# Siyou-Li/u2Tokenizer

Hardware: AMD Instinct MI355X
Metric: CT volumes/sec (256^3 fp16) through u2Tokenizer fwd (higher is better)
Workload: dtype bf16; 1 GPU; BASELINE configs[2]: u2Qwen3-8B-shaped path, 256^3 volume = 8x(32,256,256) fp16, ViT-B 3D x12, SPP, 4-layer rma+diffts+dmtp tokenizer (8 heads, top_k 1024, scales {1,2,4}, 256 queries), text 1024, prompt 1024; hidden_size=4096, batch_per_gpu=1, streams_per_gpu=2, parallelism=replicas x1, tta_side_stream=off in the multi-stream run, on in the one-stream run

## Files before the change

include/u2tok.h:

```cpp
#ifndef U2TOK_H_
#define U2TOK_H_

#include <stddef.h>
#include <stdint.h>

#ifdef __cplusplus
extern "C" {
#endif

#define U2TOK_OK 0
#define U2TOK_ERR_ARG (-1)
#define U2TOK_ERR_LAUNCH (-2)
#define U2TOK_ERR_WORKSPACE (-3)
#define U2TOK_ERR_DEVICE (-4)

typedef void* u2tok_stream_t;

int u2tok_version(void);
const char* u2tok_arch(void);
const char* u2tok_elem(void);
int u2tok_device_check(void);
typedef struct u2tok_ctx* u2tok_ctx_t;
int u2tok_ctx_create(u2tok_ctx_t* out);
int u2tok_ctx_destroy(u2tok_ctx_t ctx);
// ... 33 lines not shown
  int32_t layer_num;
} u2tok_spp_config;

typedef struct {
  int32_t B;
  int32_t T;
  int32_t N;
  int32_t E;
  int32_t Lt;
  int32_t num_heads;
  int32_t num_layers;
  int32_t top_k;
  int32_t num_query;
  int32_t use_multi_scale;
  int32_t attn_type;
  int32_t enable_diffts;
  int32_t enable_dmtp;
  int32_t max_seq_len;
  float diffts_tau;
  float ln_eps;
} u2tok_tokenizer_config;

#define U2TOK_TOK_NW(layers) (1 + 18 * (layers) + 4 + 33 * (layers) + 9)


size_t u2tok_vit_workspace_bytes(const u2tok_vit_config* cfg);
int u2tok_vit_forward(const u2tok_vit_config* cfg, const void* const* weights, const void* volume, void* out,
                      void* workspace, size_t workspace_bytes, u2tok_stream_t stream);

size_t u2tok_spp_workspace_bytes(const u2tok_spp_config* cfg);
int u2tok_spp_forward(const u2tok_spp_config* cfg, const void* const* weights, const void* x, void* out,
                      void* workspace, size_t workspace_bytes, u2tok_stream_t stream);

size_t u2tok_tokenizer_workspace_bytes(const u2tok_tokenizer_config* cfg);
int u2tok_tokenizer_forward(const u2tok_tokenizer_config* cfg, const void* const* weights, const void* v_token,
                            const void* t_token, void* out, int64_t* topk_idx_out, void* svr_out, void* workspace,
                            size_t workspace_bytes, u2tok_stream_t stream);

typedef struct {
  const void* const* svr_in;
  void* const* svr_out;
  const void* visual_in;
  void* visual_out;
  const void* const* tta_in;
  void* const* tta_out;
} u2tok_tokenizer_taps;
int u2tok_tokenizer_forward_taps(const u2tok_tokenizer_config* cfg, const void* const* weights, const void* v_token,
                                 const void* t_token, void* out, int64_t* topk_idx_out, const u2tok_tokenizer_taps* taps,
                                 void* workspace, size_t workspace_bytes, u2tok_stream_t stream);

int u2tok_embed_splice(const void* table, const int64_t* ids, const void* feats, void* out, int32_t B, int32_t S,
                       int32_t E, int32_t nfeat, int64_t vocab, u2tok_stream_t stream);

size_t u2tok_preprocess_workspace_bytes(int32_t D, int32_t H, int32_t W);
int u2tok_preprocess_volume(const float* vol, void* out, int32_t* info, int32_t D, int32_t H, int32_t W, int32_t target,
                            int32_t depth_pad, float lower_pct, float upper_pct, int32_t out_dtype, void* workspace,
                            size_t workspace_bytes, u2tok_stream_t stream);

typedef struct {
  int32_t rot90_k;
// ... 252 lines not shown
```

u2tokenizer_amd/_lib.py:

```python
from __future__ import annotations

import ctypes as C
import os
import subprocess
import threading
from pathlib import Path

_PKG = Path(__file__).resolve().parent
_LIB = _PKG / "lib" / "libu2tok_hip.so"
_LIBS = {"bf16": _LIB, "f16": _PKG / "lib" / "libu2tok_hip_f16.so"}
_lock = threading.Lock()
_handles = {}


class LibraryNotBuilt(RuntimeError):
    pass


def lib_path() -> Path:
    return _LIB


def build(verbose: bool = False) -> Path:
    cmd = ["make", "-C", str(_PKG / "csrc"), "-j", str(os.cpu_count() or 4)]
# ... 72 lines not shown
_vp, _i32, _i64, _f32, _sz = C.c_void_p, C.c_int32, C.c_int64, C.c_float, C.c_size_t

SIGNATURES = {
    "u2tok_version": (_i32, []),
    "u2tok_arch": (C.c_char_p, []),
    "u2tok_elem": (C.c_char_p, []),
    "u2tok_device_check": (_i32, []),
    "u2tok_ctx_create": (_i32, [C.POINTER(_vp)]),
    "u2tok_ctx_destroy": (_i32, [_vp]),
    "u2tok_ctx_set_current": (_i32, [_vp]),
    "u2tok_ctx_get_current": (_vp, []),
    "u2tok_set_option": (_i32, [C.c_char_p, _i32]),
    "u2tok_profile_collect": (_i32, [_vp, _vp, _vp, _i32]),
    "u2tok_profile_collect2": (_i32, [_vp, _vp, _vp, _vp, _i32]),
    "u2tok_set_gemm_scratch": (_i32, [_vp, _sz, _vp]),
    "u2tok_vit_workspace_bytes": (_sz, [C.POINTER(VitConfig)]),
    "u2tok_vit_forward": (_i32, [C.POINTER(VitConfig), C.POINTER(_vp), _vp, _vp, _vp, _sz, _vp]),
    "u2tok_spp_workspace_bytes": (_sz, [C.POINTER(SppConfig)]),
    "u2tok_spp_forward": (_i32, [C.POINTER(SppConfig), C.POINTER(_vp), _vp, _vp, _vp, _sz, _vp]),
    "u2tok_tokenizer_workspace_bytes": (_sz, [C.POINTER(TokConfig)]),
    "u2tok_tokenizer_forward": (_i32, [C.POINTER(TokConfig), C.POINTER(_vp), _vp, _vp, _vp, _vp, _vp, _vp, _sz, _vp]),
    "u2tok_tokenizer_forward_taps": (_i32, [C.POINTER(TokConfig), C.POINTER(_vp), _vp, _vp, _vp, _vp, C.POINTER(TokTaps),
                                            _vp, _sz, _vp]),
    "u2tok_tok_attention_workspace_bytes": (_sz, [_i32, _i32, _i32, _i32, _i32]),
    "u2tok_tok_attention": (_i32, [_vp, _vp, _vp, _vp, _i32, _i32, _i32, _i32, _i32, _i64, _i64, _i64, _i64, _i64, _i64, _i64,
                                   _i64, _f32, _vp, _i32, _i32, _vp, _sz, _vp]),
    "u2tok_preprocess_workspace_bytes": (_sz, [_i32, _i32, _i32]),
    "u2tok_preprocess_volume": (_i32, [_vp, _vp, _vp, _i32, _i32, _i32, _i32, _i32, _f32, _f32, _i32, _vp, _sz, _vp]),
    "u2tok_preprocess_volume_aug": (_i32, [_vp, _vp, _vp, _i32, _i32, _i32, _i32, _i32, _f32, _f32, _i32,
                                           C.POINTER(Augment), _vp, _sz, _vp]),
    "u2tok_embed_splice": (_i32, [_vp, _vp, _vp, _vp, _i32, _i32, _i32, _i32, _i64, _vp]),
    "u2tok_gemm_bf16": (_i32, [_vp, _vp, _vp, _vp, _vp, _i32, _i32, _i32, _i64, _i64, _i64, _i64, _i32, _i32,
                               _i64, _i64, _i64, _i64, _i64, _i64, _i64, _i64, _f32, _i32, _vp]),
    "u2tok_layernorm_bf16": (_i32, [_vp, _vp, _vp, _vp, _vp, _i32, _i32, _f32, _vp]),
    "u2tok_layernorm_rows": (_i32, [_vp, _vp, _vp, _vp, _vp, _i32, _i32, _i32, _i64, _i64, _i64, _i64, _i64, _i64, _f32, _vp]),
    "u2tok_softmax_rows": (_i32, [_vp, _vp, _i32, _i32, _i32, _i64, _i64, _f32, _vp, _i32, _i32, _vp]),
    "u2tok_transpose_bf16": (_i32, [_vp, _vp, _i32, _i32, _i32, _i64, _i64, _i64, _i64, _i32, _vp]),
    "u2tok_im2col_patches": (_i32, [_vp, _i32, _vp, _i32, _i32, _i32, _i32, _i32, _i32, _i32, _vp]),
    "u2tok_avgpool3d_tokens": (_i32, [_vp, _vp, _i32, _i32, _i32, _i32, _i32, _i32, _i32, _i32, _vp]),
    "u2tok_score_gemv": (_i32, [_vp, _vp, _vp, _vp, _i32, _i32, _vp]),
    "u2tok_topk_sorted": (_i32, [_vp, _vp, _i32, _i32, _i32, _vp]),
    "u2tok_gather_rows": (_i32, [_vp, _vp, _vp, _i32, _i32, _i32, _i32, _vp]),
    "u2tok_multiscale_pool": (_i32, [_vp, _vp, _i32, _i32, _i32, _vp, _vp, _vp, _vp]),
    "u2tok_temporal_attention": (_i32, [_vp, _vp, _vp, _vp, _i32, _i32, _i32, _i32, _i32, _i64, _i64, _f32, _vp,
                                        _i32, _vp]),
    "u2tok_flash_attention_d64": (_i32, [_vp, _vp, _vp, _vp, _i32, _i32, _i32, _i64, _i64, _i64, _i64, _i32, _f32,
# ... 131 lines not shown
```

u2tokenizer_amd/csrc/capi.hip:

```cpp
#include <math.h>
#include <string.h>
#include <new>
#include <vector>
#include "pipeline.h"

using namespace u2;

static_assert(U2TOK_OK == U2_OK && U2TOK_ERR_ARG == U2_ERR_ARG && U2TOK_ERR_LAUNCH == U2_ERR_LAUNCH &&
                  U2TOK_ERR_WORKSPACE == U2_ERR_WORKSPACE && U2TOK_ERR_DEVICE == U2_ERR_DEVICE,
              "public and internal status codes must agree");

#define BF(p) reinterpret_cast<const bf16_t*>(p)
#define BFW(p) reinterpret_cast<bf16_t*>(p)
#define ST(s) reinterpret_cast<hipStream_t>(s)

extern "C" {

int u2tok_version(void) { return 200;  }
const char* u2tok_arch(void) { return "gfx950"; }
const char* u2tok_elem(void) { return U2_ELEM_ASM; }

int u2tok_device_check(void) {
  int dev = 0;
  if (hipGetDevice(&dev) != hipSuccess) return U2_ERR_DEVICE;
// ... 14 lines not shown
  delete cx;
  return U2_OK;
}
int u2tok_ctx_set_current(u2tok_ctx_t c) {
  ctx_bind(reinterpret_cast<Context*>(c));
  return U2_OK;
}
u2tok_ctx_t u2tok_ctx_get_current(void) { return reinterpret_cast<u2tok_ctx_t>(ctx_bound()); }

int u2tok_set_option(const char* name, int value) {
  if (!name) return U2_ERR_ARG;
  Options& o = ctx().opt;
  struct Opt { const char* name; int Options::*field; int lo, hi; };
  static const Opt table[] = {
      {"gemm_splitk", &Options::gemm_splitk, -1, 16},   {"gemm_mubuf", &Options::gemm_mubuf, 0, 1}, {"ln_wide", &Options::ln_wide, 0, 1},   {"gemm_big", &Options::gemm_big, -1, 27},
      {"gemm_big_grid", &Options::gemm_big_grid, 1, 4096}, {"gemm_big_splitk", &Options::gemm_big_splitk, 0, 16},
      {"gemm_big_drain", &Options::gemm_big_drain, 0, 1}, {"gemm_skinny", &Options::gemm_skinny, 0, 2},
       {"kmajor_b", &Options::kmajor_b, 0, 1},            {"gemm_tail_fused", &Options::gemm_tail_fused, 0, 1},
      {"flash_mode", &Options::flash_mode, 0, 7},        {"flash_q_prescaled", &Options::flash_q_prescaled, 0, 1},
      {"vit_flash", &Options::vit_flash, 0, 1},         {"tta_overlap", &Options::tta_overlap, 0, 1},
      {"vit_vt_epilogue", &Options::vit_vt_epilogue, 0, 1},
      {"tok_flash", &Options::tok_flash, 0, 1},
      {"tok_wide", &Options::tok_wide, 0, 2},
  };
  if (!strcmp(name, "gemm_tile")) {
    if (value != 0 && value != 64 && value != 128) return U2_ERR_ARG;
    o.gemm_tile = value;
    return U2_OK;
  }
  if (!strcmp(name, "profile")) { prof_enable(value != 0); return U2_OK; }
  for (const Opt& t : table)
    if (!strcmp(name, t.name)) {
      if (value < t.lo || value > t.hi) return U2_ERR_ARG;
      if (t.field == &Options::gemm_big && value > 0 && !(value >= 20 && value <= 27 && value != 23 && value != 25)) return U2_ERR_ARG;
      if (t.field == &Options::flash_mode && value != 0 && value != 1 && value != 7) return U2_ERR_ARG;
      o.*(t.field) = value;
      return U2_OK;
    }
  return U2_ERR_ARG;
}

int u2tok_set_gemm_scratch(void* device_ptr, size_t bytes, void* stream) {
  ctx().set_scratch(reinterpret_cast<hipStream_t>(stream), device_ptr, device_ptr ? bytes : 0);
  return U2_OK;
}

// ... 31 lines not shown
}

size_t u2tok_tokenizer_workspace_bytes(const u2tok_tokenizer_config* cfg) {
  if (!cfg) return 0;
  size_t peak = 0;
  if (tokenizer_forward(*cfg, nullptr, nullptr, nullptr, nullptr, nullptr, nullptr, nullptr, nullptr, 0, true, &peak,
                        nullptr) != U2_OK)
    return 0;
  return peak + 256;
}
int u2tok_tokenizer_forward(const u2tok_tokenizer_config* cfg, const void* const* weights, const void* v_token,
                            const void* t_token, void* out, int64_t* topk_idx_out, void* svr_out, void* workspace,
                            size_t workspace_bytes, u2tok_stream_t stream) {
  if (!cfg || !workspace || ((uintptr_t)workspace & 255)) return U2_ERR_ARG;
  return tokenizer_forward(*cfg, weights, BF(v_token), BF(t_token), BFW(out), topk_idx_out, BFW(svr_out), nullptr, workspace,
                           workspace_bytes, false, nullptr, ST(stream));
}
int u2tok_tokenizer_forward_taps(const u2tok_tokenizer_config* cfg, const void* const* weights, const void* v_token,
                                 const void* t_token, void* out, int64_t* topk_idx_out, const u2tok_tokenizer_taps* taps,
                                 void* workspace, size_t workspace_bytes, u2tok_stream_t stream) {
  if (!cfg || !taps || !workspace || ((uintptr_t)workspace & 255)) return U2_ERR_ARG;
  return tokenizer_forward(*cfg, weights, BF(v_token), BF(t_token), BFW(out), topk_idx_out, nullptr, taps, workspace,
                           workspace_bytes, false, nullptr, ST(stream));
}

size_t u2tok_preprocess_workspace_bytes(int32_t D, int32_t H, int32_t W) { return preprocess_workspace_bytes(D, H, W); }
int u2tok_preprocess_volume(const float* vol, void* out, int32_t* info, int32_t D, int32_t H, int32_t W, int32_t target,
                            int32_t depth_pad, float lower_pct, float upper_pct, int32_t out_dtype, void* workspace,
                            size_t workspace_bytes, u2tok_stream_t stream) {
  return preprocess_volume(vol, out, info, D, H, W, target, depth_pad, lower_pct, upper_pct, out_dtype, nullptr, workspace,
                           workspace_bytes, ST(stream));
}
int u2tok_preprocess_volume_aug(const float* vol, void* out, int32_t* info, int32_t D, int32_t H, int32_t W, int32_t target,
                                int32_t depth_pad, float lower_pct, float upper_pct, int32_t out_dtype,
                                const u2tok_augment* aug, void* workspace, size_t workspace_bytes, u2tok_stream_t stream) {
  if (!aug) return U2_ERR_ARG;
  PreAugment a;
  a.rot_k = aug->rot90_k;
  for (int i = 0; i < 3; ++i) a.flip[i] = aug->flip[i];
  a.mul = 1.0f + aug->scale_factor;
  a.add = aug->shift_offset;
  return preprocess_volume(vol, out, info, D, H, W, target, depth_pad, lower_pct, upper_pct, out_dtype, &a, workspace,
                           workspace_bytes, ST(stream));
}

int u2tok_embed_splice(const void* table, const int64_t* ids, const void* feats, void* out, int32_t B, int32_t S,
// ... 493 lines not shown
```

u2tokenizer_amd/csrc/ctx.h:

```cpp
#pragma once
#include <mutex>
#include <vector>
#include "common.h"

namespace u2 {

struct Options {
  int ln_wide = 1;
  int gemm_tile = 0;
  int gemm_mubuf = 1;
  int gemm_splitk = 0;
  int gemm_big = 0;
  int gemm_big_grid = 256;
  int gemm_big_splitk = 0;
  int gemm_big_drain = 1;
  int gemm_skinny = 2;
  int gemm_tail_fused = 1;
  int kmajor_b = 1;
  int flash_mode = 0;
  int flash_q_prescaled = 0;
  int vit_flash = 1;
  int vit_vt_epilogue = 1;
  int tok_flash = 1;
  int tok_wide = 2;
  int tta_overlap = 1;
  int profile = 0;
};

struct SideStream {
  hipStream_t owner = nullptr;
  hipStream_t s = nullptr;
  hipEvent_t fork = nullptr;
  hipEvent_t done[16] = {};
};

struct Scratch {
  hipStream_t st;
  void* p;
  size_t bytes;
};

struct ProfRec {
  hipEvent_t a, b;
  int cat;
  double flops, bytes;
};

struct Context {
// ... 22 lines not shown
```

u2tokenizer_amd/csrc/pipeline.h:

```cpp
#pragma once
#include <algorithm>
#include "../../include/u2tok.h"
#include "kernels.h"

namespace u2 {

typedef u2tok_vit_config VitConfig;
typedef u2tok_spp_config SppConfig;
typedef u2tok_tokenizer_config TokConfig;
typedef u2tok_tokenizer_taps TokTaps;

inline int layernorm_dense(const bf16_t* x, const bf16_t* res, const bf16_t* w, const bf16_t* b, bf16_t* y, int rows, int C,
                           float eps, hipStream_t st) {
  return layernorm_bf16(x, res, w, b, y, 1, rows, C, 0, C, 0, C, 0, C, eps, st);
}

int vit_forward(const VitConfig& c, const void* const* W, const void* volume, bf16_t* out, void* ws, size_t ws_bytes,
                bool dry, size_t* peak, hipStream_t st);
int spp_forward(const SppConfig& c, const void* const* W, const bf16_t* x, bf16_t* out, void* ws, size_t ws_bytes,
                bool dry, size_t* peak, hipStream_t st);
int tokenizer_forward(const TokConfig& c, const void* const* W, const bf16_t* v_token, const bf16_t* t_token,
                      bf16_t* out, int64_t* topk_idx_out, bf16_t* svr_out, const TokTaps* taps, void* ws, size_t ws_bytes,
                      bool dry, size_t* peak, hipStream_t st);

}
```

u2tokenizer_amd/csrc/pipeline.hip:

```cpp
#include <vector>
#include "pipeline.h"

namespace u2 {

namespace {

struct Arena {
  char* base;
  size_t cap;
  size_t off = 0, peak = 0;
  bool dry;
  Arena(void* b, size_t c, bool d) : base((char*)b), cap(c), dry(d) {}
  template <typename T>
  T* get(size_t count) {
    const size_t a = (off + 255) & ~(size_t)255;
    off = a + count * sizeof(T);
    if (off > peak) peak = off;
    if (dry) return reinterpret_cast<T*>((uintptr_t)0x1000 + a);
    return (off <= cap) ? reinterpret_cast<T*>(base + a) : nullptr;
  }
  bool ok() const { return dry || peak <= cap; }
};

struct ScratchScope {
// ... 258 lines not shown
  Arena ar(ws, ws_bytes, dry);
  const Run r{ar, dry, st};
  bf16_t* pooled = ar.get<bf16_t>((size_t)rows * c.in_dim);
  bf16_t* ha = ar.get<bf16_t>((size_t)rows * c.out_dim);
  bf16_t* hb = ar.get<bf16_t>((size_t)rows * c.out_dim);
  U2_CHECK_WS(ar);
  U2_RUN(avgpool3d_tokens(x, pooled, c.nchunk, g1, g2, g3, w1, w2, w3, c.in_dim, st));
  const bf16_t* cur = pooled;
  int cur_dim = c.in_dim;
  for (int l = 0; l < c.layer_num; ++l) {
    const bool last = (l == c.layer_num - 1);
    bf16_t* dst = last ? out : ((l & 1) ? hb : ha);
    U2_TRY(linear(r, cur, {w[2 * l], w[2 * l + 1]}, dst, c.out_dim, rows, cur_dim, c.out_dim,
                  (!last && c.layer_type == 0) ? GEMM_GELU : 0));
    cur = dst;
    cur_dim = c.out_dim;
  }
  if (peak) *peak = ar.peak;
  return U2_OK;
}

namespace {
struct Att { Lin q, k, v, o; const bf16_t* rb; };
struct SvrLayer { Att spatial, temporal; };
struct TtaLayer { Att self, visual, text; Lin norm_self, norm_v, norm_t; };
struct TokWeights {
  const bf16_t* query;
  Lin score, gate;
  Att linagg;
  std::vector<SvrLayer> svr;
  std::vector<TtaLayer> tta;
};
TokWeights tok_weights(const TokConfig& c, Table t) {
  auto att = [&](int i, bool self) {
    return Att{{t[i], t[i + 1]}, {t[i + 2], t[i + 3]}, {t[i + 4], t[i + 5]}, {t[i + 6], t[i + 7]}, self && c.attn_type == 0 ? t[i + 8] : nullptr};
  };
  const int L = c.num_layers, i_sel = 1 + 18 * L, i_tta = i_sel + 4, i_lin = i_tta + 33 * L;
  TokWeights w{t[0], {t[i_sel], t[i_sel + 1]}, {nullptr, nullptr}, att(i_lin, false), {}, {}};
  if (c.enable_dmtp) w.gate = {t[i_sel + 2], t[i_sel + 3]};
  for (int l = 0, i = 1; l < L; ++l, i += 18) w.svr.push_back({att(i, true), att(i + 9, true)});
  for (int l = 0, i = i_tta; l < L; ++l, i += 33)
    w.tta.push_back({att(i, true), att(i + 9, false), att(i + 18, false), {t[i + 27], t[i + 28]}, {t[i + 29], t[i + 30]}, {t[i + 31], t[i + 32]}});
  return w;
}

int packed_proj(const Run& r, const bf16_t* x, std::initializer_list<Lin> p, bf16_t* out, int64_t rows, int E) {
  const Lin* l = p.begin(); const int n = (int)p.size();
  bool packed = l[0].w && l[0].b;
  for (int i = 1; i < n; ++i) packed = packed && l[i].w == l[i - 1].w + (size_t)E * E && l[i].b == l[i - 1].b + E;
  if (packed) return linear(r, x, l[0], out, n * E, rows, E, n * E);
  for (int i = 0; i < n; ++i) U2_TRY(linear(r, x, l[i], out + i * E, n * E, rows, E, E));
  return U2_OK;
}
int rope_qk(const Run& r, const Heads& hd, bf16_t* qkv, int64_t n_outer, int S, int n_inner) {
  const int E = hd.H * hd.d;
  U2_RUN(rope_apply(qkv, n_outer, S, n_inner, hd.H, hd.d, 3 * E, hd.max_len, 0, r.st));
  U2_RUN(rope_apply(qkv + E, n_outer, S, n_inner, hd.H, hd.d, 3 * E, hd.max_len, 0, r.st));
  return U2_OK;
}
template <typename P> inline P* slot(P* const* per_layer, int l) { return per_layer ? per_layer[l] : nullptr; }

struct Tok {
  const TokConfig& c; Run r; const TokWeights& w;
  TokTaps taps;
  const bf16_t* t_token;
  int B, T, N, E, L, Q, k;
  Heads hd;
  int64_t rows, qrows;
  bf16_t *xa, *xb, *qkv, *sctx;
  const bf16_t* V; int Lv;
  bf16_t *qa, *qb, *qc, *qproj, *qctx, *qo;
  SideStream* side; bool overlap;
  bf16_t *kv_inline, *kv_v[8], *kv_t[8], *k_lin;

  int temporal_across_batch() {
    const size_t mark = r.ar.off;
    bf16_t* g = r.ar.get<bf16_t>((size_t)rows * 3 * E);
    bf16_t* gc = r.ar.get<bf16_t>((size_t)rows * E);
    U2_CHECK_WS(r.ar);
    const size_t S2 = (size_t)B * N;
    for (int b = 0; b < B; ++b)
      U2_TRY(copy_runs(r, g + (size_t)b * N * 3 * E, S2 * 3 * E, qkv + (size_t)b * T * N * 3 * E, (size_t)N * 3 * E, (size_t)N * 3 * E, T));
    U2_TRY(self_attention(r, hd, g, gc, T, (int)S2, 3 * E, (int64_t)S2 * 3 * E, nullptr));
    for (int b = 0; b < B; ++b)
      U2_TRY(copy_runs(r, sctx + (size_t)b * T * N * E, (size_t)N * E, gc + (size_t)b * N * E, S2 * E, (size_t)N * E, T));
    r.ar.off = mark;
    return U2_OK;
  }

  int svr_layer(int l, const bf16_t*& x) {
    const SvrLayer& a = w.svr[l];
    if (const void* in = slot(taps.svr_in, l)) x = reinterpret_cast<const bf16_t*>(in);
    bf16_t* y = (x == xa) ? xb : xa;
    U2_TRY(packed_proj(r, x, {a.spatial.q, a.spatial.k, a.spatial.v}, qkv, rows, E));
    if (c.attn_type == 1) U2_TRY(rope_qk(r, hd, qkv, (int64_t)B * T, N, 1));
    if (c.attn_type == 2)
      U2_TRY(chunk_axis_attention(r, hd, qkv, sctx, 1, B * T, N, a.spatial.rb));
    else
      U2_TRY(self_attention(r, hd, qkv, sctx, B * T, N, 3 * E, (int64_t)N * 3 * E, a.spatial.rb));
    U2_TRY(linear(r, sctx, a.spatial.o, y, E, rows, E, E));
    bf16_t* y2 = (y == xa) ? xb : xa;
    U2_TRY(packed_proj(r, y, {a.temporal.q, a.temporal.k, a.temporal.v}, qkv, rows, E));
    if (c.attn_type == 1) U2_TRY(rope_qk(r, hd, qkv, B, T, N));
    if (c.attn_type == 2 && B == 1)
      U2_TRY(self_attention(r, hd, qkv, sctx, T, N, 3 * E, (int64_t)N * 3 * E, a.temporal.rb));
    else if (c.attn_type == 2)
      U2_TRY(temporal_across_batch());
    else
      U2_TRY(chunk_axis_attention(r, hd, qkv, sctx, B, T, N, a.temporal.rb));
    U2_TRY(linear(r, sctx, a.temporal.o, y2, E, rows, E, E));
    x = y2;
    return tap(r, slot(taps.svr_out, l), x, (size_t)rows * E);
  }

  int select_diffts(const bf16_t* x, bf16_t* sel) {
    const int TN = T * N;
    const size_t mark = r.ar.off;
    const int64_t ldS = round_up(TN, 8);
    float* scT = r.ar.get<float>((size_t)B * k * ldS);
    bf16_t* P = r.ar.get<bf16_t>((size_t)B * k * ldS);
    const bool x_in_place = opts().kmajor_b && !(TN & 7);
    bf16_t* Xt = x_in_place ? nullptr : r.ar.get<bf16_t>((size_t)B * E * ldS);
    U2_CHECK_WS(r.ar);
    {
      GemmDesc g;
      g.A = w.score.w; g.B = x; g.C = scT; g.bias = w.score.b;
      g.M = k; g.N = TN; g.K = E; g.lda = E; g.ldb = E; g.ldc = ldS;
      g.nz = B; g.sBb = (int64_t)TN * E; g.sCb = (int64_t)k * ldS;
      g.flags = GEMM_BIAS_M | GEMM_OUT_F32;
      U2_RUN(gemm_bf16(g, r.st));
    }
    U2_RUN(softmax_rows(scT, P, B, k, TN, ldS, ldS, (int64_t)k * ldS, (int64_t)k * ldS, 1.0f / c.diffts_tau, nullptr, 1, 0, r.st));
    {
      GemmDesc g;
// ... 105 lines not shown
  }

  int linear_aggregation(const bf16_t* qcur, bf16_t* out) {
    U2_TRY(linear(r, qcur, w.linagg.q, qproj, E, qrows, E, E));
    if (overlap)
      U2_RUN(hip_status(hipStreamWaitEvent(r.st, side->done[2 * L], 0)));
    else
      U2_TRY(linear(r, V, w.linagg.k, k_lin, E, (int64_t)B * Lv, E, E));
    return cross_attention(r, hd, qproj, k_lin, V, E, out, B, Q, Lv);
  }
};
}

int tokenizer_forward(const TokConfig& c, const void* const* W, const bf16_t* v_token, const bf16_t* t_token,
                      bf16_t* out, int64_t* topk_idx_out, bf16_t* svr_out, const TokTaps* taps, void* ws, size_t ws_bytes,
                      bool dry, size_t* peak, hipStream_t st) {
  if (c.B <= 0 || c.T <= 0 || c.N <= 0 || c.E <= 0 || c.Lt <= 0 || c.num_heads <= 0 || c.num_layers < 0) return U2_ERR_ARG;
  if (c.E % c.num_heads || (c.E / c.num_heads) % 8 || c.top_k <= 0 || c.num_query <= 0) return U2_ERR_ARG;
  if (c.attn_type < 0 || c.attn_type > 2) return U2_ERR_ARG;
  if (!dry && (!W || !v_token || !t_token || !out)) return U2_ERR_ARG;
  const int B = c.B, E = c.E, d = E / c.num_heads, L = c.num_layers, k = c.top_k;
  if (!c.enable_diffts && k > c.T * c.N) return U2_ERR_ARG;
  if (c.N > c.max_seq_len || c.T > c.max_seq_len || c.num_query > c.max_seq_len) return U2_ERR_ARG;
  const TokWeights w = tok_weights(c, Table{dry ? nullptr : W});

  Arena ar(ws, ws_bytes, dry);
  const size_t kSplitK = std::max<size_t>(24u << 20, (size_t)16 * B * c.num_query * 3 * E);
  char* skw = ar.get<char>(kSplitK);
  U2_CHECK_WS(ar);
  ScratchScope scratch_scope(ctx(), st, skw, kSplitK, !dry);
  Tok t{c, Run{ar, dry, st}, w, (taps && !dry) ? *taps : TokTaps{}, t_token, B, c.T, c.N, E, L, c.num_query, k,
        Heads{c.num_heads, d, 1.0f / sqrtf((float)d), c.max_seq_len}, (int64_t)B * c.T * c.N, (int64_t)B * c.num_query};
  const Run& r = t.r;
  t.xa = ar.get<bf16_t>((size_t)t.rows * E);
  t.xb = ar.get<bf16_t>((size_t)t.rows * E);
  t.qkv = ar.get<bf16_t>((size_t)t.rows * 3 * E);
  t.sctx = ar.get<bf16_t>((size_t)t.rows * E);
  U2_CHECK_WS(ar);

  const bf16_t* x = v_token;
  for (int l = 0; l < L; ++l) U2_TRY(t.svr_layer(l, x));
  U2_TRY(tap(r, svr_out, x, (size_t)t.rows * E));
  bf16_t* sel = ar.get<bf16_t>((size_t)B * k * E);
  U2_CHECK_WS(ar);
  U2_TRY(c.enable_diffts ? t.select_diffts(x, sel) : t.select_topk(x, sel, topk_idx_out));
  U2_TRY(t.multiscale_pooling(sel));
  U2_TRY(t.tta_prefetch());
  U2_RUN(fill_rows(w.query, t.qa, B, (int64_t)t.Q * E, (int64_t)t.Q * E, st));
  bf16_t* qcur = t.qa;
  for (int l = 0; l < L; ++l) U2_TRY(t.tta_layer(l, qcur));
  U2_TRY(t.linear_aggregation(qcur, out));
  if (peak) *peak = ar.peak;
  U2_CHECK_WS(ar);
  return U2_OK;
}

}
```

u2tokenizer_amd/tokenizer.py:

```python
from __future__ import annotations

import ctypes as C

import torch
import torch.nn as nn

from . import _lib, ops

_ATTN_TYPES = {"rma": 0, "rope": 1}


def _init_attn(m):
    for lin in (m.wq, m.wk, m.wv, m.dense):
        nn.init.xavier_uniform_(lin.weight)
        if lin.bias is not None:
            nn.init.zeros_(lin.bias)


class RelativeMultiheadAttention(nn.Module):

    def __init__(self, d_model, num_heads, max_seq_len=512):
        super().__init__()
        assert d_model % num_heads == 0
        self.num_heads, self.d_model, self.depth, self.max_seq_len = num_heads, d_model, d_model // num_heads, max_seq_len
# ... 138 lines not shown
def _pack_qkv_linear(m) -> None:
    ws, bs = [m.wq.weight, m.wk.weight, m.wv.weight], [m.wq.bias, m.wk.bias, m.wv.bias]
    E = ws[0].shape[0]
    step_w, step_b = ws[0].numel() * ws[0].element_size(), bs[0].numel() * bs[0].element_size()
    if all(w.is_contiguous() for w in ws) and all(ws[i + 1].data_ptr() == ws[i].data_ptr() + step_w for i in (0, 1)) \
            and all(bs[i + 1].data_ptr() == bs[i].data_ptr() + step_b for i in (0, 1)):
        return
    W = torch.cat([w.data for w in ws], 0).contiguous()
    Bv = torch.cat([b.data for b in bs], 0).contiguous()
    for i in range(3):
        ws[i].data = W[i * E:(i + 1) * E]
        bs[i].data = Bv[i * E:(i + 1) * E]


def _att_ptrs(m, value_side: bool = True):
    if not value_side:
        return [m.wq.weight, m.wq.bias, m.wk.weight, m.wk.bias, None, None, None, None, None]
    if isinstance(m, nn.MultiheadAttention):
        E = m.embed_dim
        W, b = m.in_proj_weight, m.in_proj_bias
        return [W[:E], b[:E], W[E:2 * E], b[E:2 * E], W[2 * E:], b[2 * E:], m.out_proj.weight, m.out_proj.bias, None]
    return [m.wq.weight, m.wq.bias, m.wk.weight, m.wk.bias, m.wv.weight, m.wv.bias, m.dense.weight, m.dense.bias,
            getattr(m, "relative_bias", None)]


def _unshare_packed(module, state_dict, prefix, local_metadata):
    for k, v in list(state_dict.items()):
        if k.startswith(prefix) and torch.is_tensor(v) and \
                v.untyped_storage().nbytes() != v.numel() * v.element_size():
            state_dict[k] = v.detach().clone() if not v.requires_grad else v.clone().detach()
    return state_dict


class u2Tokenizer(nn.Module):

    def __init__(self, embed_size, num_heads, num_layers, top_k, use_multi_scale, num_3d_query_token, hidden_size,
                 attn_type="rma", enable_diffts=False, enable_dmtp=False):
        super().__init__()
        if embed_size != hidden_size:
            raise ValueError("embed_size must equal hidden_size (builder.py:5,11 pass config.hidden_size for both)")
        self.svt_module = SpatioTemporalVisualTokenRefinerModel(
            embed_size=embed_size, num_heads=num_heads, num_layers=num_layers, top_k=top_k,
            use_multi_scale=use_multi_scale, attn_type=attn_type, enable_diffts=enable_diffts,
            enable_dmtp=enable_dmtp)
        self.tta_module = TextConditionTokenAggregatorModel(d_model=embed_size, num_layers=num_layers,
                                                            num_heads=num_heads, attn_type=attn_type)
        self.query_tokens = nn.Parameter(torch.zeros(1, num_3d_query_token, hidden_size))
        self.query_tokens.data.normal_(mean=0.0, std=0.02)
        self.embed_size, self.num_heads, self.num_layers, self.top_k = embed_size, num_heads, num_layers, top_k
        self.use_multi_scale, self.num_query, self.attn_type = bool(use_multi_scale), num_3d_query_token, attn_type
        self.enable_diffts, self.enable_dmtp = bool(enable_diffts), bool(enable_dmtp)
        self._ws = ops._Workspace()
        self._packed_key = None
        self._dead_offloaded = False
        self._register_state_dict_hook(_unshare_packed)
        self.last_topk_indices = None
        self.capture_svr_tokens = False
        self.last_svr_tokens = None

    def _weights(self):
        w = [self.query_tokens]
        for layer in self.svt_module.attention_network.layers:
            w += _att_ptrs(layer.spatial_attention) + _att_ptrs(layer.temporal_attention)
        sn = self.svt_module.token_selection.score_net
        w += [sn.weight, sn.bias]
        if self.enable_dmtp:
            w += [self.svt_module.dynamic_pool.gate_fc.weight, self.svt_module.dynamic_pool.gate_fc.bias]
        else:
            w += [None, None]
        for layer in self.tta_module.layers_vt:
            w += _att_ptrs(layer.self_attention) + _att_ptrs(layer.visual_cross_attention) \
                + _att_ptrs(layer.text_cross_attention)
            w += [layer.norm_self.weight, layer.norm_self.bias, layer.norm_cross_v.weight, layer.norm_cross_v.bias,
                  layer.norm_cross_t.weight, layer.norm_cross_t.bias]
        w += _att_ptrs(self.tta_module.layer_linagg.linear_aggregator, value_side=False)
        return w

    def pack_weights(self) -> None:
        key = (self.query_tokens.data_ptr(), self.query_tokens.dtype)
        if self._packed_key == key:
            return
        with torch.no_grad():
            for layer in self.svt_module.attention_network.layers:
                _pack_qkv(layer.spatial_attention)
                _pack_qkv(layer.temporal_attention)
            for layer in self.tta_module.layers_vt:
                for m in (layer.self_attention, layer.visual_cross_attention, layer.text_cross_attention):
                    _pack_qkv(m)
        if self.query_tokens.is_cuda:
            torch.cuda.synchronize(self.query_tokens.device)
        self._packed_key = key

    def _apply(self, fn, *args, **kwargs):
        r = super()._apply(fn, *args, **kwargs)
        self._packed_key = None
        if self.query_tokens.is_cuda:
            self.pack_weights()
            if self._dead_offloaded:
                self.offload_dead_parameters()
        return r

    def dead_parameters(self):
        la = self.tta_module.layer_linagg.linear_aggregator
        return [la.wv.weight, la.wv.bias, la.dense.weight, la.dense.bias]

    def offload_dead_parameters(self) -> int:
        freed = 0
        for p in self.dead_parameters():
            if p.is_cuda:
                freed += p.numel() * p.element_size()
                p.data = p.data.to("cpu")
            p.requires_grad_(False)
        self._dead_offloaded = True
        return freed

    def _check_envelope(self, B, T, N, E, Lt):
        H = self.num_heads
        if E % H or (E // H) % 8:
# ... 1 lines not shown
        if max(N, T, self.num_query) > 512:
            raise RuntimeError(f"sequence lengths N={N}, T={T}, queries={self.num_query} must be <= max_seq_len = 512 "
                               "(relative-bias table / RoPE cache of the reference, rma.py:6,64-68, rope.py:19)")
        if not self.enable_diffts:
            if self.top_k > T * N:
                raise RuntimeError(f"top_k={self.top_k} > T*N={T * N}: torch.topk would raise in the reference (svr.py:82)")
            if T * N > 8192:
                raise RuntimeError(f"hard top-k sorts T*N={T * N} scores in one workgroup's LDS: limit 8192")

    def forward_with_taps(self, v_token, t_token, svr_in=None, visual_in=None, tta_in=None):
        with ops.on_device(v_token, elem=self.query_tokens.dtype):
            return self._forward_with_taps(v_token, t_token, svr_in, visual_in, tta_in)

    def _forward_with_taps(self, v_token, t_token, svr_in, visual_in, tta_in):
        h = _lib.load_library()
        self.pack_weights()
        v_token = ops._need(v_token, ops.ELEM, "v_token").contiguous()
        t_token = ops._need(t_token, ops.ELEM, "t_token").contiguous()
        (B, T, N, E) = v_token.size()
        self._check_envelope(B, T, N, E, t_token.shape[1])
        L, Q, dev = self.num_layers, self.num_query, v_token.device
        Lv = self.top_k + (self.top_k // 2 + self.top_k // 4 if self.use_multi_scale else 0)
        cfg = self._config(B, T, N, E, t_token.shape[1])
        table = ops.weight_table(self._weights())
        nbytes = h.u2tok_tokenizer_workspace_bytes(C.byref(cfg))
        keep = []

        def ptr_array(tensors, shape):
            arr = (C.c_void_p * L)()
            for i in range(L):
                t = tensors[i] if tensors is not None and i < len(tensors) else None
                if t is not None:
                    t = ops._need(t, ops.ELEM, "tap").contiguous()
                    assert tuple(t.shape) == shape, (tuple(t.shape), shape)
                    keep.append(t)
                    arr[i] = t.data_ptr()
            return arr

        svr_out = [torch.empty((B, T, N, E), dtype=ops.elem_dtype(), device=dev) for _ in range(L)]
        tta_out = [torch.empty((B, Q, E), dtype=ops.elem_dtype(), device=dev) for _ in range(L)]
        visual_out = torch.empty((B, Lv, E), dtype=ops.elem_dtype(), device=dev)
        if visual_in is not None:
            visual_in = ops._need(visual_in, ops.ELEM, "visual_in").contiguous()
            assert tuple(visual_in.shape) == (B, Lv, E)
        taps = _lib.TokTaps(svr_in=ptr_array(svr_in, (B, T, N, E)), svr_out=ptr_array(svr_out, (B, T, N, E)),
                            visual_in=None if visual_in is None else visual_in.data_ptr(), visual_out=visual_out.data_ptr(),
                            tta_in=ptr_array(tta_in, (B, Q, E)), tta_out=ptr_array(tta_out, (B, Q, E)))
# ... 4 lines not shown
            _lib.check(h.u2tok_tokenizer_forward_taps(C.byref(cfg), table, v_token.data_ptr(), t_token.data_ptr(),
                                                      out.data_ptr(), None if idx is None else idx.data_ptr(),
                                                      C.byref(taps), ws.data_ptr(), ws.numel(), stream),
                       "u2tok_tokenizer_forward_taps")
        self.last_topk_indices = idx
        return out, {"svr_out": svr_out, "visual_out": visual_out, "tta_out": tta_out}

    def _config(self, B, T, N, E, Lt):
        return _lib.TokConfig(B=B, T=T, N=N, E=E, Lt=Lt, num_heads=self.num_heads,
                              num_layers=self.num_layers, top_k=self.top_k, num_query=self.num_query,
                              use_multi_scale=int(self.use_multi_scale), attn_type=_ATTN_TYPES.get(self.attn_type, 2),
                              enable_diffts=int(self.enable_diffts), enable_dmtp=int(self.enable_dmtp),
                              max_seq_len=512, diffts_tau=float(getattr(self.svt_module.token_selection, "tau", 1.0)),
                              ln_eps=1e-5)

    def forward(self, v_token, t_token):
        with ops.on_device(v_token, elem=self.query_tokens.dtype):
            return self._forward(v_token, t_token)

    def _forward(self, v_token, t_token):
        if torch.is_grad_enabled() and (v_token.requires_grad or t_token.requires_grad
                                        or any(p.requires_grad for p in self.parameters())):
            from . import autograd as AG
            ops.training_needs_bf16(self.query_tokens.dtype, "u2Tokenizer")
            ops._need(v_token, ops.ELEM, "v_token"), ops._need(t_token, ops.ELEM, "t_token")
            (B, T, N, E) = v_token.size()
            self._check_envelope(B, T, N, E, t_token.shape[1])
            with ops.on_device(v_token):
                return AG.tokenizer_forward(self, v_token, t_token)
        h = _lib.load_library()
        if self.query_tokens.is_cuda:
            self.pack_weights()
        v_token = ops._need(v_token, ops.ELEM, "v_token").contiguous()
        t_token = ops._need(t_token, ops.ELEM, "t_token").contiguous()
        (B, T, N, E) = v_token.size()
        if E != self.embed_size or t_token.shape[0] != B or t_token.shape[2] != E:
            raise RuntimeError(f"shape mismatch: v_token {tuple(v_token.shape)}, t_token {tuple(t_token.shape)}")
        self._check_envelope(B, T, N, E, t_token.shape[1])
        cfg = self._config(B, T, N, E, t_token.shape[1])
        table = ops.weight_table(self._weights())
        nbytes = h.u2tok_tokenizer_workspace_bytes(C.byref(cfg))
        if nbytes == 0:
            raise RuntimeError("u2tok_tokenizer_workspace_bytes rejected the configuration "
                               f"(B={B}, T={T}, N={N}, E={E}, heads={self.num_heads}, top_k={self.top_k})")
        idx = svr = None
        with ops.on_device(v_token) as (h, stream):
            ws = self._ws.get(nbytes, v_token.device)
            out = torch.empty((B, self.num_query, E), dtype=ops.elem_dtype(), device=v_token.device)
            if not self.enable_diffts:
                idx = torch.empty((B, self.top_k), dtype=torch.int64, device=v_token.device)
            if self.capture_svr_tokens:
                svr = torch.empty((B, T * N, E), dtype=ops.elem_dtype(), device=v_token.device)
            _lib.check(h.u2tok_tokenizer_forward(C.byref(cfg), table, v_token.data_ptr(), t_token.data_ptr(),
                                                 out.data_ptr(), None if idx is None else idx.data_ptr(),
                                                 None if svr is None else svr.data_ptr(), ws.data_ptr(), ws.numel(),
                                                 stream), "u2tok_tokenizer_forward")
        self.last_topk_indices = idx
        self.last_svr_tokens = svr
        return out
```

Baseline: 126.5 volumes/s.

## Fold SVR output projection into the next attention's QKV projection weights

Result: faster. 134.2 volumes/s, median of 6 (+6.1%).

```diff
diff --git a/include/u2tok.h b/include/u2tok.h
--- a/include/u2tok.h
+++ b/include/u2tok.h
@@ -79,6 +79,7 @@
 } u2tok_tokenizer_config;
 
 #define U2TOK_TOK_NW(layers) (1 + 18 * (layers) + 4 + 33 * (layers) + 9)
+#define U2TOK_TOK_NFOLD(layers) ((layers) > 0 ? 2 * (2 * (layers) - 1) : 0)
 
 
 size_t u2tok_vit_workspace_bytes(const u2tok_vit_config* cfg);
@@ -93,6 +94,9 @@
 int u2tok_tokenizer_forward(const u2tok_tokenizer_config* cfg, const void* const* weights, const void* v_token,
                             const void* t_token, void* out, int64_t* topk_idx_out, void* svr_out, void* workspace,
                             size_t workspace_bytes, u2tok_stream_t stream);
+
+int u2tok_tokenizer_svr_fold(const void* w_qkv, const void* b_qkv, const void* w_o, const void* b_o, void* w_fold, void* b_fold,
+                             int32_t E, u2tok_stream_t stream);
 
 typedef struct {
   const void* const* svr_in;
diff --git a/u2tokenizer_amd/_lib.py b/u2tokenizer_amd/_lib.py
--- a/u2tokenizer_amd/_lib.py
+++ b/u2tokenizer_amd/_lib.py
@@ -118,6 +118,7 @@
     "u2tok_tokenizer_forward": (_i32, [C.POINTER(TokConfig), C.POINTER(_vp), _vp, _vp, _vp, _vp, _vp, _vp, _sz, _vp]),
     "u2tok_tokenizer_forward_taps": (_i32, [C.POINTER(TokConfig), C.POINTER(_vp), _vp, _vp, _vp, _vp, C.POINTER(TokTaps),
                                             _vp, _sz, _vp]),
+    "u2tok_tokenizer_svr_fold": (_i32, [_vp, _vp, _vp, _vp, _vp, _vp, _i32, _vp]),
     "u2tok_tok_attention_workspace_bytes": (_sz, [_i32, _i32, _i32, _i32, _i32]),
     "u2tok_tok_attention": (_i32, [_vp, _vp, _vp, _vp, _i32, _i32, _i32, _i32, _i32, _i64, _i64, _i64, _i64, _i64, _i64, _i64,
                                    _i64, _f32, _vp, _i32, _i32, _vp, _sz, _vp]),
diff --git a/u2tokenizer_amd/csrc/capi.hip b/u2tokenizer_amd/csrc/capi.hip
--- a/u2tokenizer_amd/csrc/capi.hip
+++ b/u2tokenizer_amd/csrc/capi.hip
@@ -60,6 +60,7 @@
       {"vit_vt_epilogue", &Options::vit_vt_epilogue, 0, 1},
       {"tok_flash", &Options::tok_flash, 0, 1},
       {"tok_wide", &Options::tok_wide, 0, 2},
+      {"svr_fold", &Options::svr_fold, 0, 1},
   };
   if (!strcmp(name, "gemm_tile")) {
     if (value != 0 && value != 64 && value != 128) return U2_ERR_ARG;
@@ -137,6 +138,11 @@
   if (!cfg || !taps || !workspace || ((uintptr_t)workspace & 255)) return U2_ERR_ARG;
   return tokenizer_forward(*cfg, weights, BF(v_token), BF(t_token), BFW(out), topk_idx_out, nullptr, taps, workspace,
                            workspace_bytes, false, nullptr, ST(stream));
+}
+
+int u2tok_tokenizer_svr_fold(const void* w_qkv, const void* b_qkv, const void* w_o, const void* b_o, void* w_fold, void* b_fold,
+                             int32_t E, u2tok_stream_t stream) {
+  return svr_fold_build(BF(w_qkv), BF(b_qkv), BF(w_o), BF(b_o), BFW(w_fold), BFW(b_fold), E, ST(stream));
 }
 
 size_t u2tok_preprocess_workspace_bytes(int32_t D, int32_t H, int32_t W) { return preprocess_workspace_bytes(D, H, W); }
diff --git a/u2tokenizer_amd/csrc/ctx.h b/u2tokenizer_amd/csrc/ctx.h
--- a/u2tokenizer_amd/csrc/ctx.h
+++ b/u2tokenizer_amd/csrc/ctx.h
@@ -24,6 +24,7 @@
   int tok_flash = 1;
   int tok_wide = 2;
   int tta_overlap = 1;
+  int svr_fold = 1;
   int profile = 0;
 };
 
diff --git a/u2tokenizer_amd/csrc/pipeline.h b/u2tokenizer_amd/csrc/pipeline.h
--- a/u2tokenizer_amd/csrc/pipeline.h
+++ b/u2tokenizer_amd/csrc/pipeline.h
@@ -22,5 +22,7 @@
 int tokenizer_forward(const TokConfig& c, const void* const* W, const bf16_t* v_token, const bf16_t* t_token,
                       bf16_t* out, int64_t* topk_idx_out, bf16_t* svr_out, const TokTaps* taps, void* ws, size_t ws_bytes,
                       bool dry, size_t* peak, hipStream_t st);
+int svr_fold_build(const bf16_t* Wqkv, const bf16_t* bqkv, const bf16_t* Wo, const bf16_t* bo, bf16_t* Wf, bf16_t* bf, int E,
+                   hipStream_t st);
 
 }
diff --git a/u2tokenizer_amd/csrc/pipeline.hip b/u2tokenizer_amd/csrc/pipeline.hip
--- a/u2tokenizer_amd/csrc/pipeline.hip
+++ b/u2tokenizer_amd/csrc/pipeline.hip
@@ -304,7 +304,8 @@
 
 namespace {
 struct Att { Lin q, k, v, o; const bf16_t* rb; };
-struct SvrLayer { Att spatial, temporal; };
+struct SvrAtt : Att { Lin fold; };
+struct SvrLayer { SvrAtt spatial, temporal; };
 struct TtaLayer { Att self, visual, text; Lin norm_self, norm_v, norm_t; };
 struct TokWeights {
   const bf16_t* query;
@@ -313,14 +314,26 @@
   std::vector<SvrLayer> svr;
   std::vector<TtaLayer> tta;
 };
-TokWeights tok_weights(const TokConfig& c, Table t) {
+bool packed(const Lin* l, int n, int E) {
+  bool p = l[0].w && l[0].b;
+  for (int i = 1; i < n; ++i) p = p && l[i].w == l[i - 1].w + (size_t)E * E && l[i].b == l[i - 1].b + E;
+  return p;
+}
+TokWeights tok_weights(const TokConfig& c, Table t, bool folds) {
   auto att = [&](int i, bool self) {
     return Att{{t[i], t[i + 1]}, {t[i + 2], t[i + 3]}, {t[i + 4], t[i + 5]}, {t[i + 6], t[i + 7]}, self && c.attn_type == 0 ? t[i + 8] : nullptr};
   };
-  const int L = c.num_layers, i_sel = 1 + 18 * L, i_tta = i_sel + 4, i_lin = i_tta + 33 * L;
+  const int L = c.num_layers, i_sel = 1 + 18 * L, i_tta = i_sel + 4, i_lin = i_tta + 33 * L, i_fold = U2TOK_TOK_NW(L);
+  auto svr_att = [&](int i, int j) {
+    SvrAtt a{att(i, true), {nullptr, nullptr}};
+    const Lin qkv[3] = {a.q, a.k, a.v};
+    if (folds && j > 0 && t[i_fold + 2 * (j - 1)] && t[i_fold + 2 * (j - 1) + 1] && packed(qkv, 3, c.E))
+      a.fold = {t[i_fold + 2 * (j - 1)], t[i_fold + 2 * (j - 1) + 1]};
+    return a;
+  };
   TokWeights w{t[0], {t[i_sel], t[i_sel + 1]}, {nullptr, nullptr}, att(i_lin, false), {}, {}};
   if (c.enable_dmtp) w.gate = {t[i_sel + 2], t[i_sel + 3]};
-  for (int l = 0, i = 1; l < L; ++l, i += 18) w.svr.push_back({att(i, true), att(i + 9, true)});
+  for (int l = 0, i = 1; l < L; ++l, i += 18) w.svr.push_back({svr_att(i, 2 * l), svr_att(i + 9, 2 * l + 1)});
   for (int l = 0, i = i_tta; l < L; ++l, i += 33)
     w.tta.push_back({att(i, true), att(i + 9, false), att(i + 18, false), {t[i + 27], t[i + 28]}, {t[i + 29], t[i + 30]}, {t[i + 31], t[i + 32]}});
   return w;
@@ -328,9 +341,7 @@
 
 int packed_proj(const Run& r, const bf16_t* x, std::initializer_list<Lin> p, bf16_t* out, int64_t rows, int E) {
   const Lin* l = p.begin(); const int n = (int)p.size();
-  bool packed = l[0].w && l[0].b;
-  for (int i = 1; i < n; ++i) packed = packed && l[i].w == l[i - 1].w + (size_t)E * E && l[i].b == l[i - 1].b + E;
-  if (packed) return linear(r, x, l[0], out, n * E, rows, E, n * E);
+  if (packed(l, n, E)) return linear(r, x, l[0], out, n * E, rows, E, n * E);
   for (int i = 0; i < n; ++i) U2_TRY(linear(r, x, l[i], out + i * E, n * E, rows, E, E));
   return U2_OK;
 }
@@ -350,12 +361,13 @@
   Heads hd;
   int64_t rows, qrows;
   bf16_t *xa, *xb, *qkv, *sctx;
+  bool x_ctx = false;
   const bf16_t* V; int Lv;
   bf16_t *qa, *qb, *qc, *qproj, *qctx, *qo;
   SideStream* side; bool overlap;
   bf16_t *kv_inline, *kv_v[8], *kv_t[8], *k_lin;
 
-  int temporal_across_batch() {
+  int temporal_across_batch(bf16_t* actx) {
     const size_t mark = r.ar.off;
     bf16_t* g = r.ar.get<bf16_t>((size_t)rows * 3 * E);
     bf16_t* gc = r.ar.get<bf16_t>((size_t)rows * E);
@@ -365,33 +377,46 @@
       U2_TRY(copy_runs(r, g + (size_t)b * N * 3 * E, S2 * 3 * E, qkv + (size_t)b * T * N * 3 * E, (size_t)N * 3 * E, (size_t)N * 3 * E, T));
     U2_TRY(self_attention(r, hd, g, gc, T, (int)S2, 3 * E, (int64_t)S2 * 3 * E, nullptr));
     for (int b = 0; b < B; ++b)
-      U2_TRY(copy_runs(r, sctx + (size_t)b * T * N * E, (size_t)N * E, gc + (size_t)b * N * E, S2 * E, (size_t)N * E, T));
+      U2_TRY(copy_runs(r, actx + (size_t)b * T * N * E, (size_t)N * E, gc + (size_t)b * N * E, S2 * E, (size_t)N * E, T));
     r.ar.off = mark;
+    return U2_OK;
+  }
+
+  int svr_qkv(const SvrAtt& a, const bf16_t* x) {
+    if (x_ctx) return linear(r, x, a.fold, qkv, 3 * E, rows, E, 3 * E);
+    return packed_proj(r, x, {a.q, a.k, a.v}, qkv, rows, E);
+  }
+  bf16_t* svr_ctx(const bf16_t* x) const { return x == sctx ? xa : sctx; }
+  int svr_project(const SvrAtt& a, const SvrAtt* next, bf16_t* actx, const bf16_t*& x) {
+    x_ctx = next && next->fold.w;
+    if (x_ctx) { x = actx; return U2_OK; }
+    bf16_t* y = (x == xa || actx == xa) ? xb : xa;
+    U2_TRY(linear(r, actx, a.o, y, E, rows, E, E));
+    x = y;
     return U2_OK;
   }
 
   int svr_layer(int l, const bf16_t*& x) {
     const SvrLayer& a = w.svr[l];
     if (const void* in = slot(taps.svr_in, l)) x = reinterpret_cast<const bf16_t*>(in);
-    bf16_t* y = (x == xa) ? xb : xa;
-    U2_TRY(packed_proj(r, x, {a.spatial.q, a.spatial.k, a.spatial.v}, qkv, rows, E));
+    bf16_t* actx = svr_ctx(x);
+    U2_TRY(svr_qkv(a.spatial, x));
     if (c.attn_type == 1) U2_TRY(rope_qk(r, hd, qkv, (int64_t)B * T, N, 1));
     if (c.attn_type == 2)
-      U2_TRY(chunk_axis_attention(r, hd, qkv, sctx, 1, B * T, N, a.spatial.rb));
+      U2_TRY(chunk_axis_attention(r, hd, qkv, actx, 1, B * T, N, a.spatial.rb));
     else
-      U2_TRY(self_attention(r, hd, qkv, sctx, B * T, N, 3 * E, (int64_t)N * 3 * E, a.spatial.rb));
-    U2_TRY(linear(r, sctx, a.spatial.o, y, E, rows, E, E));
-    bf16_t* y2 = (y == xa) ? xb : xa;
-    U2_TRY(packed_proj(r, y, {a.temporal.q, a.temporal.k, a.temporal.v}, qkv, rows, E));
+      U2_TRY(self_attention(r, hd, qkv, actx, B * T, N, 3 * E, (int64_t)N * 3 * E, a.spatial.rb));
+    U2_TRY(svr_project(a.spatial, &a.temporal, actx, x));
+    actx = svr_ctx(x);
+    U2_TRY(svr_qkv(a.temporal, x));
     if (c.attn_type == 1) U2_TRY(rope_qk(r, hd, qkv, B, T, N));
     if (c.attn_type == 2 && B == 1)
-      U2_TRY(self_attention(r, hd, qkv, sctx, T, N, 3 * E, (int64_t)N * 3 * E, a.temporal.rb));
+      U2_TRY(self_attention(r, hd, qkv, actx, T, N, 3 * E, (int64_t)N * 3 * E, a.temporal.rb));
     else if (c.attn_type == 2)
-      U2_TRY(temporal_across_batch());
+      U2_TRY(temporal_across_batch(actx));
     else
-      U2_TRY(chunk_axis_attention(r, hd, qkv, sctx, B, T, N, a.temporal.rb));
-    U2_TRY(linear(r, sctx, a.temporal.o, y2, E, rows, E, E));
-    x = y2;
+      U2_TRY(chunk_axis_attention(r, hd, qkv, actx, B, T, N, a.temporal.rb));
+    U2_TRY(svr_project(a.temporal, l + 1 < L ? &w.svr[l + 1].spatial : nullptr, actx, x));
     return tap(r, slot(taps.svr_out, l), x, (size_t)rows * E);
   }
 
@@ -543,7 +568,9 @@
   const int B = c.B, E = c.E, d = E / c.num_heads, L = c.num_layers, k = c.top_k;
   if (!c.enable_diffts && k > c.T * c.N) return U2_ERR_ARG;
   if (c.N > c.max_seq_len || c.T > c.max_seq_len || c.num_query > c.max_seq_len) return U2_ERR_ARG;
-  const TokWeights w = tok_weights(c, Table{dry ? nullptr : W});
+  bool folds = !dry && opts().svr_fold && !svr_out;
+  for (int l = 0; folds && taps && l < L; ++l) folds = !slot(taps->svr_in, l) && !slot(taps->svr_out, l);
+  const TokWeights w = tok_weights(c, Table{dry ? nullptr : W}, folds);
 
   Arena ar(ws, ws_bytes, dry);
   const size_t kSplitK = std::max<size_t>(24u << 20, (size_t)16 * B * c.num_query * 3 * E);
@@ -576,4 +603,18 @@
   return U2_OK;
 }
 
-}
+int svr_fold_build(const bf16_t* Wqkv, const bf16_t* bqkv, const bf16_t* Wo, const bf16_t* bo, bf16_t* Wf, bf16_t* bf, int E,
+                   hipStream_t st) {
+  if (!Wqkv || !bqkv || !Wo || !bo || !Wf || !bf || E <= 0 || (E & 7)) return U2_ERR_ARG;
+  if (Wf == Wqkv || Wf == Wo || bf == bqkv || bf == bo) return U2_ERR_ARG;
+  ScratchScope scratch_scope(ctx(), st, nullptr, 0, true);
+  GemmDesc g;
+  g.A = Wqkv; g.B = Wo; g.C = Wf;
+  g.M = 3 * E; g.N = E; g.K = E;
+  g.lda = E; g.ldb = E; g.ldc = E;
+  g.flags = GEMM_B_KMAJOR;
+  U2_TRY(gemm_bf16(g, st));
+  return gemm_bf16(linear_desc(bo, E, Wqkv, bqkv, bf, 3 * E, 1, E, 3 * E, 0, nullptr, 0), st);
+}
+
+}
diff --git a/u2tokenizer_amd/tokenizer.py b/u2tokenizer_amd/tokenizer.py
--- a/u2tokenizer_amd/tokenizer.py
+++ b/u2tokenizer_amd/tokenizer.py
@@ -184,6 +184,24 @@
         return [W[:E], b[:E], W[E:2 * E], b[E:2 * E], W[2 * E:], b[2 * E:], m.out_proj.weight, m.out_proj.bias, None]
     return [m.wq.weight, m.wq.bias, m.wk.weight, m.wk.bias, m.wv.weight, m.wv.bias, m.dense.weight, m.dense.bias,
             getattr(m, "relative_bias", None)]
+
+
+def _fold_sources(m):
+    if isinstance(m, nn.MultiheadAttention):
+        return (m.in_proj_weight, m.in_proj_bias, m.out_proj.weight, m.out_proj.bias), \
+            [m.in_proj_weight, m.in_proj_bias, m.out_proj.weight, m.out_proj.bias]
+    return (m.wq.weight, m.wq.bias, m.dense.weight, m.dense.bias), \
+        [m.wq.weight, m.wq.bias, m.wk.weight, m.wk.bias, m.wv.weight, m.wv.bias, m.dense.weight, m.dense.bias]
+
+
+def _qkv_packed(m) -> bool:
+    if isinstance(m, nn.MultiheadAttention):
+        return m.in_proj_weight is not None and m.in_proj_bias is not None and m.out_proj.bias is not None
+    ws, bs = [m.wq.weight, m.wk.weight, m.wv.weight], [m.wq.bias, m.wk.bias, m.wv.bias]
+    if any(b is None for b in bs) or m.dense.bias is None:
+        return False
+    sw, sb = ws[0].numel() * ws[0].element_size(), bs[0].numel() * bs[0].element_size()
+    return all(ws[i + 1].data_ptr() == ws[i].data_ptr() + sw and bs[i + 1].data_ptr() == bs[i].data_ptr() + sb for i in (0, 1))
 
 
 def _unshare_packed(module, state_dict, prefix, local_metadata):
@@ -214,6 +232,8 @@
         self.enable_diffts, self.enable_dmtp = bool(enable_diffts), bool(enable_dmtp)
         self._ws = ops._Workspace()
         self._packed_key = None
+        self._folds = None
+        self._fold_key = None
         self._dead_offloaded = False
         self._register_state_dict_hook(_unshare_packed)
         self.last_topk_indices = None
@@ -240,22 +260,66 @@
 
     def pack_weights(self) -> None:
         key = (self.query_tokens.data_ptr(), self.query_tokens.dtype)
-        if self._packed_key == key:
+        repacked = self._packed_key != key
+        if repacked:
+            with torch.no_grad():
+                for layer in self.svt_module.attention_network.layers:
+                    _pack_qkv(layer.spatial_attention)
+                    _pack_qkv(layer.temporal_attention)
+                for layer in self.tta_module.layers_vt:
+                    for m in (layer.self_attention, layer.visual_cross_attention, layer.text_cross_attention):
+                        _pack_qkv(m)
+            self.invalidate_folds()
+        if self.query_tokens.is_cuda:
+            refold = self._fold_key is None or self._fold_key != self._fold_versions()
+            if refold:
+                self._build_folds()
+            if refold or repacked:
+                torch.cuda.synchronize(self.query_tokens.device)
+        self._packed_key = key
+
+    def invalidate_folds(self) -> None:
+        self._folds = self._fold_key = None
+
+    def _svr_chain(self):
+        return [m for layer in self.svt_module.attention_network.layers
+                for m in (layer.spatial_attention, layer.temporal_attention)]
+
+    def _fold_versions(self):
+        return tuple(p._version for m in self._svr_chain() for p in _fold_sources(m)[1])
+
+    def _build_folds(self) -> None:
+        chain, dt, dev = self._svr_chain(), self.query_tokens.dtype, self.query_tokens.device
+        self._folds, self._fold_key = None, self._fold_versions()
+        if len(chain) < 2 or dt not in ops.ELEM_OF:
             return
-        with torch.no_grad():
-            for layer in self.svt_module.attention_network.layers:
-                _pack_qkv(layer.spatial_attention)
-                _pack_qkv(layer.temporal_attention)
-            for layer in self.tta_module.layers_vt:
-                for m in (layer.self_attention, layer.visual_cross_attention, layer.text_cross_attention):
-                    _pack_qkv(m)
-        if self.query_tokens.is_cuda:
-            torch.cuda.synchronize(self.query_tokens.device)
-        self._packed_key = key
+        E, n = self.embed_size, len(chain) - 1
+        with torch.no_grad(), ops.on_device(self.query_tokens, elem=dt) as (h, stream):
+            W = torch.empty((n, 3 * E, E), dtype=dt, device=dev)
+            b = torch.empty((n, 3 * E), dtype=dt, device=dev)
+            folds = []
+            for j in range(1, len(chain)):
+                if not _qkv_packed(chain[j]):
+                    folds.append(None)
+                    continue
+                (w_qkv, b_qkv, _, _), _ = _fold_sources(chain[j])
+                (_, _, w_o, b_o), _ = _fold_sources(chain[j - 1])
+                _lib.check(h.u2tok_tokenizer_svr_fold(w_qkv.data_ptr(), b_qkv.data_ptr(), w_o.data_ptr(), b_o.data_ptr(),
+                                                      W[j - 1].data_ptr(), b[j - 1].data_ptr(), E, stream),
+                           "u2tok_tokenizer_svr_fold")
+                folds.append((W[j - 1], b[j - 1]))
+        self._folds = folds
+
+    def _fold_slots(self):
+        n = max(0, 2 * self.num_layers - 1)
+        if self._folds is None:
+            return [None] * (2 * n)
+        return [t for f in self._folds for t in (f if f is not None else (None, None))]
 
     def _apply(self, fn, *args, **kwargs):
         r = super()._apply(fn, *args, **kwargs)
         self._packed_key = None
+        self.invalidate_folds()
         if self.query_tokens.is_cuda:
             self.pack_weights()
             if self._dead_offloaded:
@@ -303,7 +367,7 @@
         L, Q, dev = self.num_layers, self.num_query, v_token.device
         Lv = self.top_k + (self.top_k // 2 + self.top_k // 4 if self.use_multi_scale else 0)
         cfg = self._config(B, T, N, E, t_token.shape[1])
-        table = ops.weight_table(self._weights())
+        table = ops.weight_table(self._weights() + self._fold_slots())
         nbytes = h.u2tok_tokenizer_workspace_bytes(C.byref(cfg))
         keep = []
 
@@ -354,6 +418,7 @@
         if torch.is_grad_enabled() and (v_token.requires_grad or t_token.requires_grad
                                         or any(p.requires_grad for p in self.parameters())):
             from . import autograd as AG
+            self.invalidate_folds()
             ops.training_needs_bf16(self.query_tokens.dtype, "u2Tokenizer")
             ops._need(v_token, ops.ELEM, "v_token"), ops._need(t_token, ops.ELEM, "t_token")
             (B, T, N, E) = v_token.size()
@@ -370,7 +435,7 @@
             raise RuntimeError(f"shape mismatch: v_token {tuple(v_token.shape)}, t_token {tuple(t_token.shape)}")
         self._check_envelope(B, T, N, E, t_token.shape[1])
         cfg = self._config(B, T, N, E, t_token.shape[1])
-        table = ops.weight_table(self._weights())
+        table = ops.weight_table(self._weights() + self._fold_slots())
         nbytes = h.u2tok_tokenizer_workspace_bytes(C.byref(cfg))
         if nbytes == 0:
             raise RuntimeError("u2tok_tokenizer_workspace_bytes rejected the configuration "
```
